# douglasbagnall/recur

Hardware: AMD Instinct MI355X
Metric: BPTT timesteps*streams/sec at 1024-hidden/256-stream (higher is better)
Workload: dtype f32; 1 GPU; text-predict multi-tap generation: hidden 1024, 256 streams/GPU, BPTT depth 20, 42 symbols, RELU, weighted momentum, lr 1e-5; streams_per_gpu=256, global_streams=256, scaling_mode=weak, parallelism=single GPU, rccl_ranks=0, exchange=none

## Files before the change

### recur_amd/csrc/k_delta_direct.h

```cpp
#pragma once
#include <hip/hip_runtime.h>
#include <stdint.h>
#include <utility>
#include "k_tiles.h"

typedef float dd_f4 __attribute__((ext_vector_type(4)));
typedef float dd_f4u __attribute__((ext_vector_type(4), aligned(4)));

struct DdArgs {
  const float *x;
  const float *e;
  const float *coef;
  const int *n_exec;
  const float *ih_scale;
  float *w, *m, *delta;
  size_t plane;
  int I, H, Scap;
  int nrows, D, uidx;
  int tm, tn;
  int rest;
  int hidden_size;
  int mode;
  int method;
  float rate, momentum, mw;
  float *ho_w, *ho_m;
  const float *ho_delta;
  float *ho_delta_out;
  unsigned ho_n4;
  float ho_rate;
  int ksplit;
  size_t kplane;
  int rgroups;
  int ho_ks;
  size_t ho_plane;
  int fast_its;
};

template <bool COLD = false> __device__ __forceinline__ dd_f4 dd_load4(const void *sbase, unsigned voff) {
  dd_f4 r;
  if constexpr (COLD) asm volatile("s_nop 4\n\tglobal_load_dwordx4 %0, %1, %2" : "=v"(r) : "v"(voff), "s"(sbase) : "memory");
  else asm volatile("global_load_dwordx4 %0, %1, %2" : "=v"(r) : "v"(voff), "s"(sbase) : "memory");
  return r;
}
template <bool COLD = false> __device__ __forceinline__ float dd_load1(const void *sbase, unsigned voff) {
  float r;
  if constexpr (COLD) asm volatile("s_nop 4\n\tglobal_load_dword %0, %1, %2" : "=v"(r) : "v"(voff), "s"(sbase) : "memory");
  else asm volatile("global_load_dword %0, %1, %2" : "=v"(r) : "v"(voff), "s"(sbase) : "memory");
  return r;
}
typedef int dd_i4 __attribute__((ext_vector_type(4)));
__device__ __forceinline__ dd_i4 dd_load4i(const void *sbase, unsigned voff) {
  dd_i4 r;
  asm volatile("s_nop 4\n\tglobal_load_dwordx4 %0, %1, %2" : "=v"(r) : "v"(voff), "s"(sbase) : "memory");
  return r;
}
template <int N> __device__ __forceinline__ void dd_flag_wait(dd_i4 (&n)[DD_FLAG_LOADS / 2], dd_f4 (&s)[DD_FLAG_LOADS / 2]) {
  static_assert(DD_FLAG_LOADS == 8, "operand list");
  asm volatile("s_waitcnt vmcnt(%8)" : "+v"(n[0]), "+v"(n[1]), "+v"(n[2]), "+v"(n[3]), "+v"(s[0]), "+v"(s[1]), "+v"(s[2]), "+v"(s[3]) : "n"(N));
}
template <int N> __device__ __forceinline__ void dd_wait3(dd_f4 &a, dd_f4 &b, float &c) {
  asm volatile("s_waitcnt vmcnt(%3)" : "+v"(a), "+v"(b), "+v"(c) : "n"(N));
}
template <int N> __device__ __forceinline__ void dd_wait4(dd_f4 &a, dd_f4 &b, float &c, float &d) {
  asm volatile("s_waitcnt vmcnt(%4)" : "+v"(a), "+v"(b), "+v"(c), "+v"(d) : "n"(N));
}
template <int N> __device__ __forceinline__ void dd_wait5(dd_f4 &a, dd_f4 &b, float &c, float &d, float &e) {
  asm volatile("s_waitcnt vmcnt(%5)" : "+v"(a), "+v"(b), "+v"(c), "+v"(d), "+v"(e) : "n"(N));
}
template <int N> __device__ __forceinline__ void dd_wait6(dd_f4 &a, dd_f4 &b, float &c, float &d, float &e, float &f) {
  asm volatile("s_waitcnt vmcnt(%6)" : "+v"(a), "+v"(b), "+v"(c), "+v"(d), "+v"(e), "+v"(f) : "n"(N));
}
template <int N> __device__ __forceinline__ void dd_wait7(dd_f4 &a, dd_f4 &b, float &c, float &d, float &e, float &f, float &g) {
  asm volatile("s_waitcnt vmcnt(%7)" : "+v"(a), "+v"(b), "+v"(c), "+v"(d), "+v"(e), "+v"(f), "+v"(g) : "n"(N));
}
template <int P> __device__ __forceinline__ void dd_drain(const dd_f4 (&a)[P], const dd_f4 (&b)[P], const float (&c)[2][P], const float (&s)[2][P], const float (&d)[P]) {
  static_assert(P == 5, "operand list");
  asm volatile("s_waitcnt vmcnt(0)"
               :
               : "v"(a[0]), "v"(a[1]), "v"(a[2]), "v"(a[3]), "v"(a[4]), "v"(b[0]), "v"(b[1]), "v"(b[2]), "v"(b[3]), "v"(b[4]),
                 "v"(c[0][0]), "v"(c[0][1]), "v"(c[0][2]), "v"(c[0][3]), "v"(c[0][4]), "v"(c[1][0]), "v"(c[1][1]), "v"(c[1][2]),
                 "v"(c[1][3]), "v"(c[1][4]), "v"(s[0][0]), "v"(s[0][1]), "v"(s[0][2]), "v"(s[0][3]), "v"(s[0][4]), "v"(s[1][0]), "v"(s[1][1]),
                 "v"(s[1][2]), "v"(s[1][3]), "v"(s[1][4]), "v"(d[0]), "v"(d[1]), "v"(d[2]), "v"(d[3]), "v"(d[4])
               : "memory");
}
template <int... Is, class F>
__device__ __forceinline__ void dd_static_for_impl(std::integer_sequence<int, Is...>, F &&f) {
  (f(std::integral_constant<int, Is>{}), ...);
}
template <int N, class F> __device__ __forceinline__ void dd_static_for(F &&f) {
  dd_static_for_impl(std::make_integer_sequence<int, N>{}, f);
}

constexpr int DD_LD = 64;
#ifndef DD_NT_STORES
#define DD_NT_STORES 1
#endif
template <int LEVEL> __device__ __forceinline__ void dd_store4(float *p, const float __attribute__((ext_vector_type(4))) & v) {
  typedef float f4u __attribute__((ext_vector_type(4), aligned(4)));
  if constexpr (DD_NT_STORES >= LEVEL) __builtin_nontemporal_store(v, reinterpret_cast<f4u *>(p));
  else *reinterpret_cast<f4u *>(p) = v;
}

#ifdef PC_STAMPS
__device__ unsigned long long g_ddir_stamps[4][8];
__device__ unsigned long long g_ddir_wave[4][8];
__device__ unsigned long long g_ddir_clk[4][4];
#define DDIR_CLOCKS(i) do { if ((blockIdx.x & 63) == 0 && threadIdx.x == 0) { g_ddir_clk[blockIdx.x >> 6][i] = __builtin_amdgcn_s_memrealtime(); g_ddir_clk[blockIdx.x >> 6][(i) + 1] = __builtin_amdgcn_s_memtime(); } } while (0)
#define DDIR_STAMP(i) do { if ((blockIdx.x & 63) == 0 && threadIdx.x == 0) g_ddir_stamps[blockIdx.x >> 6][i] = __builtin_amdgcn_s_memrealtime(); } while (0)
#else
#define DDIR_STAMP(i) do { } while (0)
#define DDIR_CLOCKS(i) do { } while (0)
#endif
struct DdNoPre {
  __device__ __forceinline__ void operator()() const {}
};
template <int NW, int P, int NPW, class PRE = DdNoPre>
__device__ __forceinline__ void dd_body(const DdArgs &a, float *lds, PRE pre = PRE{}) {
  const int wv = __builtin_amdgcn_readfirstlane((int)(threadIdx.x >> 6)), lane = threadIdx.x & 63;
  DDIR_STAMP(0);
  const int ksp = a.ksplit > 1 ? a.ksplit : 1, per_part = gridDim.x / ksp;
  const int kz = (int)blockIdx.x / per_part;
  const int L = (int)blockIdx.x - kz * per_part, xcd = L & 7, q = L >> 3;
  float *const dlt = a.delta + (size_t)kz * a.kplane;
  int mt, nt;
  if ((a.tm & 3) == 0 && (a.tn & 1) == 0) {
    const int bm = a.tm >> 2, bn = a.tn >> 1;
    mt = (xcd & 3) * bm + q % bm;
    nt = (xcd >> 2) * bn + q / bm;
  } else {
    mt = L % a.tm;
    nt = L / a.tm;
  }
  if (nt >= a.tn) return;
  const int m0 = 64 * mt, n0 = 64 * nt;
  const int I = a.I;
  const int QPS = a.nrows >> 2;
  constexpr int ST = NW / 2;
  const int n_pair = 2 * (a.D * (QPS / NW) / ksp);
  const int nf = a.fast_its > 0 ? a.fast_its : n_pair / 2;
  const bool first_of_pair = wv < ST;
  const int n_it = first_of_pair ? nf : n_pair - nf;
  const int q0 = (wv & (ST - 1)) + ST * (kz * n_pair + (first_of_pair ? 0 : nf));
  const int g_t0 = q0 / QPS, g_w0 = q0 - g_t0 * QPS;
  const unsigned voff = (unsigned)(((size_t)(lane >> 4) * I + (lane & 15) * 4) * sizeof(float));
  const int RG = a.rgroups;
  const bool has_rest = a.rest > 0 && NPW * mt < 4 * RG;
  const int rg = (a.rest + RG - 1) / RG;
  int ri[NPW], rj[NPW], rrows[NPW];
  unsigned voff_r[NPW];
  unsigned voff_s[NPW];
#pragma unroll
  for (int p = 0; p < NPW; p++) {
    const int pi = has_rest ? NPW * mt + p : 0;
    ri[p] = pi >> 2;
    rj[p] = pi & 3;
    int left = a.rest - ri[p] * rg;
    rrows[p] = has_rest ? (left < 0 ? 0 : left < rg ? left : rg) : 0;
    const int c = lane & 15;
    const int rcol = rrows[p] > 0 ? 64 * a.tm - m0 + ri[p] * rg + (c < rrows[p] ? c : rrows[p] - 1) : 0;
    voff_r[p] = (unsigned)(((size_t)(lane >> 4) * I + rcol) * sizeof(float));
    voff_s[p] = voff + (unsigned)(rj[p] * sizeof(float));
  }
  const unsigned voff_c = (unsigned)((lane >> 4) * sizeof(float));

  constexpr int CPT = 1024 / (64 * NW);
  const bool upd = a.mode == 2;

  dd_f4 fl_s[DD_FLAG_LOADS / 2];
  dd_i4 fl_n[DD_FLAG_LOADS / 2];
#pragma unroll
  for (int u = 0; u < DD_FLAG_LOADS / 2; u++) {
    int r4 = 4 * (64 * u + lane);
    r4 = r4 < a.nrows ? r4 : a.nrows - 4;
    fl_n[u] = dd_load4i(a.n_exec, (unsigned)(r4 * sizeof(int)));
    fl_s[u] = dd_load4<true>(a.ih_scale, (unsigned)(r4 * sizeof(float)));
  }

  dd_f4 ra[P], re[P];
  float rr[2][P], rs[2][P], rcf[P];
  int g_t = g_t0, g_within = g_w0;
  const float *g_xb, *g_eb, *g_cb;
  auto advance = [&]() {
    const int t = g_t < a.D ? g_t : a.D - 1;
    int slot = a.uidx - t;
    slot = slot < 0 ? slot + a.D : slot;
    const size_t ro = (size_t)(g_within << 2) * I;
    g_xb = a.x + (size_t)slot * a.plane + ro + m0;
    g_eb = a.e + (size_t)t * a.plane + ro + n0;
    g_cb = a.coef + (size_t)t * a.Scap + (g_within << 2);
    const int over = g_within + ST - QPS, neg = over >> 31;
    g_within = over + (neg & QPS);
    g_t += 1 + neg;
  };
  dd_f4 acc[4][4], racc[NPW];
#pragma unroll
  for (int p = 0; p < NPW; p++) racc[p] = dd_f4{0.f, 0.f, 0.f, 0.f};
#pragma unroll
  for (int j = 0; j < P; j++) rr[1][j] = rs[1][j] = 0.0f;
#pragma unroll
  for (int i = 0; i < 4; i++)
#pragma unroll
    for (int j = 0; j < 4; j++) acc[i][j] = dd_f4{0.f, 0.f, 0.f, 0.f};
  dd_static_for<P>([&](auto JC) {
    constexpr int j = decltype(JC)::value;
    advance();
    ra[j] = dd_load4<true>(g_xb, voff);
    re[j] = dd_load4<true>(g_eb, voff);
#pragma unroll
    for (int p = 0; p < NPW; p++) {
      rr[p][j] = dd_load1<true>(g_xb, voff_r[p]);
      rs[p][j] = dd_load1<true>(g_eb, voff_s[p]);
    }
  });
  pre();
  int ones;
  {
    DDIR_STAMP(1);
    dd_flag_wait<(2 + 2 * NPW) * P>(fl_n, fl_s);
    DDIR_STAMP(2);
    DDIR_CLOCKS(0);
    bool ok = true;
#pragma unroll
    for (int u = 0; u < DD_FLAG_LOADS / 2; u++)
#pragma unroll
      for (int k = 0; k < 4; k++) ok = ok && fl_n[u][k] == a.D && fl_s[u][k] == 1.0f;
    ones = __builtin_amdgcn_readfirstlane(__all(ok) ? 1 : 0);
  }
  auto round = [&](auto ONESC) {
    constexpr bool ONES = decltype(ONESC)::value;
    dd_static_for<P>([&](auto JC) {
      constexpr int j = decltype(JC)::value;
      constexpr int PER = 2 + 2 * NPW + (ONES ? 0 : 1);
      if constexpr (ONES && NPW == 1) dd_wait4<PER * (P - 1)>(ra[j], re[j], rr[0][j], rs[0][j]);
      else if constexpr (ONES) dd_wait6<PER * (P - 1)>(ra[j], re[j], rr[0][j], rr[1][j], rs[0][j], rs[1][j]);
      else if constexpr (NPW == 1) dd_wait5<PER * (P - 1)>(ra[j], re[j], rr[0][j], rs[0][j], rcf[j]);
      else dd_wait7<PER * (P - 1)>(ra[j], re[j], rr[0][j], rr[1][j], rs[0][j], rs[1][j], rcf[j]);
      dd_f4 fa = ra[j], fe = re[j];
      float fr[NPW], fsel[NPW];
#pragma unroll
      for (int p = 0; p < NPW; p++) {
        fr[p] = rr[p][j];
        fsel[p] = rs[p][j];
      }
      if constexpr (!ONES) {
        if constexpr (NPW == 1)
          asm volatile("v_mul_legacy_f32 %0, %5, %0\n\tv_mul_legacy_f32 %1, %5, %1\n\t"
                       "v_mul_legacy_f32 %2, %5, %2\n\tv_mul_legacy_f32 %3, %5, %3\n\tv_mul_legacy_f32 %4, %5, %4\n\ts_nop 1"
                       : "+v"(fe[0]), "+v"(fe[1]), "+v"(fe[2]), "+v"(fe[3]), "+v"(fsel[0])
                       : "v"(rcf[j]));
        else
          asm volatile("v_mul_legacy_f32 %0, %6, %0\n\tv_mul_legacy_f32 %1, %6, %1\n\t"
                       "v_mul_legacy_f32 %2, %6, %2\n\tv_mul_legacy_f32 %3, %6, %3\n\tv_mul_legacy_f32 %4, %6, %4\n\t"
                       "v_mul_legacy_f32 %5, %6, %5\n\ts_nop 1"
                       : "+v"(fe[0]), "+v"(fe[1]), "+v"(fe[2]), "+v"(fe[3]), "+v"(fsel[0]), "+v"(fsel[NPW - 1])
                       : "v"(rcf[j]));
      }
      __builtin_amdgcn_sched_barrier(0);
      advance();
#pragma unroll
      for (int i = 0; i < 4; i++)
#pragma unroll
        for (int jn = 0; jn < 4; jn++)
          acc[i][jn] = __builtin_amdgcn_mfma_f32_16x16x4f32(fa[i], fe[jn], acc[i][jn], 0, 0, 0);
#pragma unroll
      for (int p = 0; p < NPW; p++) racc[p] = __builtin_amdgcn_mfma_f32_16x16x4f32(fr[p], fsel[p], racc[p], 0, 0, 0);
#pragma unroll
      for (int g = 0; g < 16 + NPW; g++) {
        __builtin_amdgcn_sched_group_barrier(0x008, 1, 0);
        __builtin_amdgcn_sched_group_barrier(0x004, 4, 0);
      }
      __builtin_amdgcn_sched_barrier(0);
      ra[j] = dd_load4(g_xb, voff);
      re[j] = dd_load4(g_eb, voff);
#pragma unroll
      for (int p = 0; p < NPW; p++) {
        rr[p][j] = dd_load1(g_xb, voff_r[p]);
        rs[p][j] = dd_load1(g_eb, voff_s[p]);
      }
      if constexpr (!ONES) rcf[j] = dd_load1(g_cb, voff_c);
      __builtin_amdgcn_sched_barrier(0);
    });
  };
  if (ones) {
    for (int i0 = 0; i0 < n_it; i0 += P) round(std::true_type{});
    DDIR_STAMP(3);
    DDIR_CLOCKS(2);
#ifdef PC_STAMPS
    if ((blockIdx.x & 63) == 0 && lane == 0) g_ddir_wave[blockIdx.x >> 6][wv] = __builtin_amdgcn_s_memrealtime();
#endif
#pragma unroll
    for (int j = 0; j < P; j++) rcf[j] = 0.0f;
    dd_drain<P>(ra, re, rr, rs, rcf);
  } else {
#pragma unroll
    for (int j = 0; j < P; j++) rcf[j] = 0.0f;
    dd_drain<P>(ra, re, rr, rs, rcf);
    g_t = g_t0;
    g_within = g_w0;
    dd_static_for<P>([&](auto JC) {
      constexpr int j = decltype(JC)::value;
      advance();
      ra[j] = dd_load4<true>(g_xb, voff);
      re[j] = dd_load4<true>(g_eb, voff);
#pragma unroll
      for (int p = 0; p < NPW; p++) {
        rr[p][j] = dd_load1<true>(g_xb, voff_r[p]);
        rs[p][j] = dd_load1<true>(g_eb, voff_s[p]);
      }
      rcf[j] = dd_load1<true>(g_cb, voff_c);
    });
    for (int i0 = 0; i0 < n_it; i0 += P) round(std::false_type{});
    dd_drain<P>(ra, re, rr, rs, rcf);
  }

  {
    float *base = lds + (size_t)wv * 64 * DD_LD;
#pragma unroll
    for (int i = 0; i < 4; i++)
#pragma unroll
      for (int r = 0; r < 4; r++) {
        const int row = 16 * (lane >> 4) + 4 * r + i;
        *reinterpret_cast<dd_f4 *>(base + row * DD_LD + 4 * (lane & 15)) = dd_f4{acc[i][0][r], acc[i][1][r], acc[i][2][r], acc[i][3][r]};
      }
#pragma unroll
    for (int p = 0; p < NPW; p++) {
      float *rb = lds + (size_t)NW * 64 * DD_LD + (p * NW + wv) * 256;
#pragma unroll
      for (int r = 0; r < 4; r++) rb[(4 * (lane >> 4) + r) * 16 + (lane & 15)] = racc[p][r];
    }
  }
  DDIR_STAMP(4);
  __syncthreads();
  DDIR_STAMP(5);
  const bool adagrad = a.method == 4;
  auto update4 = [&](dd_f4 &W, dd_f4 &M, const dd_f4 &d, float rate) {
#pragma unroll
    for (int k = 0; k < 4; k++) {
      if (adagrad) {
        const float acc2 = M[k] + d[k] * d[k];
        W[k] += d[k] * rate / sqrtf(acc2);
        M[k] = acc2;
      } else {
        const float t = d[k] * rate, mm = M[k];
        W[k] += t + mm * a.mw;
        M[k] = (mm + t) * a.momentum;
      }
    }
  };
#pragma unroll
  for (int u = 0; u < CPT; u++) {
    const int ch = u * 64 * NW + threadIdx.x;
    const float *p = lds + (ch >> 4) * DD_LD + 4 * (ch & 15);
    dd_f4 s = *reinterpret_cast<const dd_f4 *>(p);
#pragma unroll
    for (int w2 = 1; w2 < NW; w2++) s += *reinterpret_cast<const dd_f4 *>(p + (size_t)w2 * 64 * DD_LD);
    const size_t off = (size_t)(m0 + (ch >> 4)) * a.H + n0 + 4 * (ch & 15);
    if (a.mode == 1) s += *reinterpret_cast<const dd_f4u *>(dlt + off);
    dd_store4<1>(dlt + off, s);
    if (upd) {
      dd_f4 W = *reinterpret_cast<const dd_f4u *>(a.w + off), M = *reinterpret_cast<const dd_f4u *>(a.m + off);
      update4(W, M, s, a.rate);
      dd_store4<2>(a.w + off, W);
      dd_store4<1>(a.m + off, M);
    }
  }
  auto update1 = [&](size_t off, float d, float rate, float *w, float *m) {
    if (adagrad) {
      const float acc2 = m[off] + d * d;
      w[off] += d * rate / sqrtf(acc2);
      m[off] = acc2;
      return;
    }
    const float t = d * rate, mm = m[off];
    w[off] += t + mm * a.mw;
    m[off] = (mm + t) * a.momentum;
  };
  if (has_rest && threadIdx.x < 256 * NPW) {
    const int p = threadIdx.x >> 8, t8 = threadIdx.x & 255;
    const int c = t8 >> 4, c2 = t8 & 15;
    const int pri = NPW == 1 ? ri[0] : (p ? ri[NPW - 1] : ri[0]), prj = NPW == 1 ? rj[0] : (p ? rj[NPW - 1] : rj[0]);
    const int prows = NPW == 1 ? rrows[0] : (p ? rrows[NPW - 1] : rrows[0]);
    if (c < prows) {
      const float *q = lds + (size_t)NW * 64 * DD_LD + (size_t)p * NW * 256 + t8;
      float d = q[0];
#pragma unroll
      for (int w2 = 1; w2 < NW; w2++) d += q[w2 * 256];
      const size_t off = (size_t)(64 * a.tm + pri * rg + c) * a.H + n0 + 4 * c2 + prj;
      if (a.mode == 1) d += dlt[off];
      dlt[off] = d;
      if (upd) update1(off, d, a.rate, a.w, a.m);
    }
  }
  const int hi_cols = a.H - a.hidden_size - 1;
  if (a.mode != 1 && (nt == 0 || nt == a.tn - 1)) {
    const int ncol = nt == 0 && nt == a.tn - 1 ? 1 + hi_cols : nt == 0 ? 1 : hi_cols;
    const int nrow = 64 + (mt == 0 ? a.rest : 0);
    for (int e = threadIdx.x; e < nrow * ncol; e += 64 * NW) {
      const int rr_ = e / ncol, cc = e - rr_ * ncol;
      const int row = rr_ < 64 ? m0 + rr_ : 64 * a.tm + rr_ - 64;
      const int col = (nt == 0 && cc == 0) ? -1 : a.hidden_size + (nt == 0 ? cc - 1 : cc);
      const ptrdiff_t off = (ptrdiff_t)row * a.H + col;
      dlt[off] = 0.0f;
      if (upd && adagrad) {
        a.w[off] += 0.0f * a.rate / sqrtf(a.m[off]);
      } else if (upd) {
        const float mm = a.m[off];
        a.w[off] += mm * a.mw;
        a.m[off] = mm * a.momentum;
      }
    }
  }
  if (upd && a.ho_n4) {
    const unsigned per = (a.ho_n4 + gridDim.x - 1) / gridDim.x;
    for (unsigned k = threadIdx.x; k < per; k += 64 * NW) {
      const unsigned idx = blockIdx.x * per + k;
      if (idx >= a.ho_n4) break;
      const size_t off = 4 * (size_t)idx;
      dd_f4 d = *reinterpret_cast<const dd_f4 *>(a.ho_delta + off);
      for (int z = 1; z < a.ho_ks; z++) {
        const dd_f4 t = *reinterpret_cast<const dd_f4 *>(a.ho_delta + (size_t)z * a.ho_plane + off);
        d[0] += t[0]; d[1] += t[1]; d[2] += t[2]; d[3] += t[3];
      }
      if (a.ho_delta_out) *reinterpret_cast<dd_f4 *>(a.ho_delta_out + off) = d;
      dd_f4 W = *reinterpret_cast<const dd_f4 *>(a.ho_w + off), M = *reinterpret_cast<const dd_f4 *>(a.ho_m + off);
      update4(W, M, d, a.ho_rate);
      *reinterpret_cast<dd_f4 *>(a.ho_w + off) = W;
      *reinterpret_cast<dd_f4 *>(a.ho_m + off) = M;
    }
  }
  DDIR_STAMP(6);
}

constexpr int dd_lds_bytes(int NW, int NPW = 1) { return (NW * 64 * DD_LD + NPW * NW * 256) * 4; }

#ifndef DD_BND_MARK
#define DD_BND_MARK(which) do { } while (0)
#endif
template <int NW, int P, int NPW = 1>
__global__ __launch_bounds__(64 * NW) __attribute__((amdgpu_waves_per_eu(NW / 4, NW / 4))) void k_delta_direct(DdArgs a) {
  extern __shared__ __attribute__((aligned(16))) float dd_lds[];
  __builtin_amdgcn_s_setprio(2);
  DD_BND_MARK(0);
  dd_body<NW, P, NPW>(a, dd_lds);
  DD_BND_MARK(1);
}
```

### recur_amd/csrc/kernels_bptt.hip

```cpp
#include "k_common.h"
#include "k_gemm.h"
#include "calc_plan.h"

__global__ __launch_bounds__(64) void k_bottom_error(View v, int row0, int nxp,
                                                     const unsigned char *active) {
  const RamdShape &s = v.sh;
  int j = blockIdx.x, r = row0 + j;
  int n = (active && !active[j]) ? 0 : v.b.n_exec[r];
  for (int y = threadIdx.x; y < s.bO; y += 64) {
    float sum = 0.0f;
    if (y < s.input_size)
      for (int k = 0; k < n; k++) sum += v.b.ex[((size_t)(k + 1) * s.Scap + r) * nxp + y + 1];
    v.b.berr[(size_t)r * s.bO + y] = sum;
  }
}

__global__ __launch_bounds__(256) void k_bottom_delta(View v, int row0, int nrows, int accumulate,
                                                      const unsigned char *active,
                                                      const float *carry_in, float *carry_out) {
  const RamdShape &s = v.sh;
  int e = blockIdx.x * 256 + threadIdx.x;
  if (e >= s.bI * s.bO) return;
  int yi = e / s.bO, x = e - yi * s.bO;
  float cum = carry_in[x];
  float acc = accumulate ? v.b.bdelta[e] : 0.0f;
  for (int j = 0; j < nrows; j++) {
    if (active && !active[j]) continue;
    int r = row0 + j;
    cum += v.b.berr[(size_t)r * s.bO + x];
    const float sc = v.b.ih_scale[r];
    if (sc != 1.0f && x < s.input_size) cum *= sc * sc;
    float xi = v.b.binp[(size_t)r * s.bI + yi];
    if (xi != 0.0f) acc += xi * cum;
  }
  v.b.bdelta[e] = acc;
  if (yi == 0) carry_out[x] = cum;
}

#include "k_bptt_top.h"
#include "k_bptt_extras.h"

BND_DECL(g_bnd_delta, ramd_bnd_delta_stamps)
#ifdef BND_STAMPS
#define DD_BND_MARK(which) BND_MARK(g_bnd_delta, which)
#endif
#include "k_delta_direct.h"

#ifdef PC_STAMPS
extern "C" void ramd_ddir_stamps(unsigned long long *out) {
  HIP_CHECK(hipDeviceSynchronize());
  HIP_CHECK(hipMemcpyFromSymbol(out, HIP_SYMBOL(g_ddir_stamps), sizeof(unsigned long long) * 32));
  HIP_CHECK(hipMemcpyFromSymbol(out + 32, HIP_SYMBOL(g_ddir_wave), sizeof(unsigned long long) * 32));
}
extern "C" void ramd_ddir_clocks(unsigned long long *out) {
  HIP_CHECK(hipDeviceSynchronize());
  HIP_CHECK(hipMemcpyFromSymbol(out, HIP_SYMBOL(g_ddir_clk), sizeof(unsigned long long) * 16));
}
#endif
template <int NW, int P, int NPW>
__global__ __launch_bounds__(64 * NW) __attribute__((amdgpu_waves_per_eu(NW / 4, NW / 4))) void k_delta_direct_ho(DdArgs a, View v,
                                                                                                                HoWork hw, HoApply ap) {
  extern __shared__ __attribute__((aligned(16))) float ddh_lds[];
  __builtin_amdgcn_s_setprio(2);
  BND_MARK(g_bnd_delta, 0);
#ifndef DD_HO_AT_END
#define DD_HO_AT_END 1
#endif
#if DD_HO_AT_END
  dd_body<NW, P, NPW>(a, ddh_lds);
  __syncthreads();
  chain_ho_delta<5, 8>(v, hw, ddh_lds, (int)blockIdx.x, ap);
#else
  dd_body<NW, P, NPW>(a, ddh_lds, [&]() { chain_ho_delta<5, 8>(v, hw, ddh_lds, (int)blockIdx.x, ap); });
#endif
  BND_MARK(g_bnd_delta, 1);
}

#include "k_delta_dma.h"
#include "k_bptt_small.h"


__global__ __launch_bounds__(256) void k_delta_finalize(float *delta, const float *slab,
                                                        size_t n4, size_t n, int ks,
                                                        int accumulate, int H, int hidden_size,
                                                        int rows_core, int ks_rest,
                                                        const float *rest, size_t rest_stride,
                                                        float *ho_delta, const float *ho_slab,
                                                        size_t ho_n, int ho_ks) {
  size_t q = (size_t)blockIdx.x * 256 + threadIdx.x;
  const size_t ih_threads = ((n4 + 255) / 256) * 256;
  if (q >= ih_threads) {
    size_t e = q - ih_threads;
    if (ho_slab && 4 * e < ho_n) {
      float4 a = accumulate ? ld4(ho_delta + 4 * e) : zero4();
      for (int z = 0; z < ho_ks; z++) {
        float4 t = ld4(ho_slab + (size_t)z * ho_n + 4 * e);
        a.x += t.x; a.y += t.y; a.z += t.z; a.w += t.w;
      }
      *reinterpret_cast<float4 *>(ho_delta + 4 * e) = a;
    }
    return;
  }
  if (q >= n4) return;
  const float *src = slab + 4 * q;
  size_t stride = n;
  if ((int)((4 * q) / (size_t)H) >= rows_core) {
    ks = ks_rest;
    src = rest + (4 * q - (size_t)rows_core * H);
    stride = rest_stride;
  }
  float4 a = accumulate ? ld4(delta + 4 * q) : zero4();
  float4 sum = sum_planes(src, stride, ks);
  int c = (int)((4 * q) % (size_t)H);
  a.x += (c + 0 >= 1 && c + 0 <= hidden_size) ? sum.x : 0.0f;
  a.y += (c + 1 >= 1 && c + 1 <= hidden_size) ? sum.y : 0.0f;
  a.z += (c + 2 >= 1 && c + 2 <= hidden_size) ? sum.z : 0.0f;
  a.w += (c + 3 >= 1 && c + 3 <= hidden_size) ? sum.w : 0.0f;
  *reinterpret_cast<float4 *>(delta + 4 * q) = a;
}

extern "C" void ramd_launch_pending_finalize(ramd_stream_t st_, const RamdPendingDelta *p) {
  hipStream_t st = (hipStream_t)st_;
  const size_t n4 = p->slab ? p->n / 4 : 0;
  const unsigned blocks = (unsigned)((n4 + 255) / 256) + (p->ho_slab ? (unsigned)((p->ho_n / 4 + 255) / 256) : 0u);
  if (!blocks) return;
  RAMD_LAUNCH(k_delta_finalize, dim3(blocks), dim3(256), 0, st, p->delta_out, p->slab, n4, p->n, p->ks, 0, p->H,
              p->hidden_size, p->rows_core, p->ks_rest, p->rest, p->rest_stride, p->ho_delta_out, p->ho_slab, p->ho_n,
              p->ho_ks);
}

__global__ __launch_bounds__(256) void k_err_writeback(View v, int row0, int nxp) {
  int r = row0 + blockIdx.x;
  int n = v.b.n_exec[r];
  if (n <= 0) return;
  for (int i = threadIdx.x; i < v.sh.I; i += 256) write_error_images(v, r, n, nxp, i);
}

__global__ void k_zero_f4(float *a, size_t n4) {
  size_t q = (size_t)blockIdx.x * blockDim.x + threadIdx.x;
  if (q < n4) *reinterpret_cast<float4 *>(a + 4 * q) = zero4();
}

extern "C" void ramd_launch_bottom_deltas(ramd_stream_t st_, const RamdShape *sh, RamdBuffers *b,
                                          int row0, int nrows, int accumulate,
                                          const unsigned char *active) {
  hipStream_t st = (hipStream_t)st_;
  View v = make_view(sh, b);
  RAMD_LAUNCH(k_bottom_error, dim3(nrows), dim3(64), 0, st, v, row0, ramd_nxp(sh), active);
  int n = sh->bI * sh->bO;
  const float *cin = b->bcarry + (size_t)b->bcarry_cur * sh->bO;
  float *cout = b->bcarry + (size_t)(b->bcarry_cur ^ 1) * sh->bO;
  RAMD_LAUNCH(k_bottom_delta, dim3((n + 255) / 256), dim3(256), 0, st, v, row0, nrows,
                     accumulate, active, cin, cout);
  b->bcarry_cur ^= 1;
}

extern "C" void ramd_launch_clear_deltas(ramd_stream_t st_, const RamdShape *sh,
                                         const RamdBuffers *b) {
  hipStream_t st = (hipStream_t)st_;
  size_t ih4 = (size_t)sh->I * sh->H / 4, ho4 = (size_t)sh->H * sh->O / 4;
  RAMD_LAUNCH(k_zero_f4, dim3((unsigned)((ih4 + 255) / 256)), dim3(256), 0, st, b->ih_delta, ih4);
  RAMD_LAUNCH(k_zero_f4, dim3((unsigned)((ho4 + 255) / 256)), dim3(256), 0, st, b->ho_delta, ho4);
  if (sh->bI) {
    size_t b4 = (size_t)sh->bI * sh->bO / 4, c4 = (size_t)2 * sh->bO / 4;
    RAMD_LAUNCH(k_zero_f4, dim3((unsigned)((b4 + 255) / 256)), dim3(256), 0, st, b->bdelta, b4);
    RAMD_LAUNCH(k_zero_f4, dim3((unsigned)((c4 + 255) / 256)), dim3(256), 0, st, b->bcarry, c4);
  }
}

static int g_calc_wrote_images = 0;
static void (*g_delta_half_hook)(void *ctx, int half, size_t first_float, size_t n_floats) = nullptr;
static void *g_delta_half_ctx = nullptr;
extern "C" void ramd_set_delta_half_hook(void (*hook)(void *, int, size_t, size_t), void *ctx) {
  g_delta_half_hook = hook;
  g_delta_half_ctx = ctx;
}
extern "C" int ramd_calc_wrote_images(void) {
  int w = g_calc_wrote_images;
  g_calc_wrote_images = 0;
  return w;
}

struct CalcCall {
  hipStream_t st;
  View v;
  const RamdShape *sh;
  const RamdBuffers *b;
  int row0, nrows, accumulate;
  const int *ranges;
  int range_stride;
  const unsigned char *active;
  RamdPendingDelta *defer;
  CalcPlan p;
};

static void calc_top_backprop(const CalcCall &c) {
  const RamdShape *sh = c.sh;
  const RamdBuffers *b = c.b;
  const CalcPlan &p = c.p;
  if (p.writeback_first) ramd_launch_err_writeback(c.st, sh, b, c.row0, c.nrows);
  const size_t shm = (size_t)(sh->O + sh->H) * sizeof(float);
  if (p.top == TOP_SPARSE) {
    const int alen = b->mheads_alen, ncls = sh->output_size / alen;
    const int span4 = (3 + alen + 3) / 4, ld = (4 * span4) | 1;
    raise_lds_limit<k_top_heads_partial>(96 * 1024);
    RAMD_LAUNCH(k_top_heads_partial, dim3(ncls, (sh->H + THP_ROWS - 1) / THP_ROWS), dim3(256),
                (size_t)((THP_ROWS + 32) * ld + 4) * sizeof(float), c.st, c.v, c.row0, c.nrows, c.ranges, c.range_stride, c.active,
                alen, ncls, b->mheads_part);
    RAMD_LAUNCH(k_top_heads_combine, dim3(c.nrows), dim3(THC_THREADS), 0, c.st, c.v, c.row0, c.ranges, c.range_stride, c.active,
                ncls, b->mheads_part, (p.flags & RAMD_IMAGES_PENDING) ? 1 : 0);
  } else if (p.top == TOP_HEADS) {
    const int tm = (c.nrows + 31) / 32, tn = (sh->H + 31) / 32;
    RAMD_LAUNCH(k_top_backprop_heads, dim3(tm * tn), dim3(512), (size_t)((sh->O + 15) / 16) * sizeof(unsigned), c.st, c.v,
                c.row0, c.nrows, c.ranges, c.range_stride, c.active, b->slab, p.top_nb, tm);
    RAMD_LAUNCH(k_top_backprop_scale, dim3(c.nrows), dim3(256), 0, c.st, c.v, c.row0, c.active, b->slab, p.top_nb);
  } else if (p.top == TOP_RANGED) {
    RAMD_LAUNCH(k_top_backprop_ranged, dim3(c.nrows, p.top_nb), dim3(1024), shm, c.st, c.v, c.row0, c.ranges, c.range_stride,
                c.active, b->slab);
    if (p.top_nb > 1) RAMD_LAUNCH(k_top_backprop_scale, dim3(c.nrows), dim3(256), 0, c.st, c.v, c.row0, c.active, b->slab, p.top_nb);
  } else if (p.top == TOP_PLAIN)
    RAMD_LAUNCH(k_top_backprop, dim3(c.nrows), dim3(256), shm, c.st, c.v, c.row0, c.ranges, c.range_stride, c.active);
}

struct HoOwed {
  bool gemm, sum_here;
  ProbHoDelta prob;
  int nkt, ks;
};

static HoOwed calc_top_delta(const CalcCall &c, HoWork *req, bool chain_answered) {
  const RamdShape *sh = c.sh;
  const RamdBuffers *b = c.b;
  RamdPendingDelta *defer = c.defer;
  HoOwed owed = {};
  if (c.p.ho_in_delta || (c.p.flags & RAMD_NO_HO_DELTA)) return owed;
  if (c.p.ho_asked && !chain_answered) {
    req->dst = (defer && b->ho_slab) ? b->ho_slab : b->ho_delta;
    req->active = c.active;
    req->row0 = c.row0;
    req->nrows = c.nrows;
    return owed;
  }
  if (c.p.ho_asked && req->done) {
    if (defer) {
      defer->ho_slab = req->dst == b->ho_slab ? b->ho_slab : nullptr;
      defer->ho_n = (size_t)sh->H * sh->O;
      defer->ho_ks = 1;
      defer->ho_delta_out = b->ho_delta;
    }
    return owed;
  }
  const HoGemmPlan h = ramd_plan_ho_gemm(sh, b, c.p, c.nrows, c.accumulate, c.ranges != nullptr, c.range_stride,
                                         c.active != nullptr, defer != nullptr);
  if (defer) defer->ho_slab = nullptr;
  if (h.form == HO_HEADS) {
    const int alen = b->mheads_alen, ncls = sh->output_size / alen;
    RAMD_LAUNCH(k_ho_delta_heads, dim3(ncls, (sh->H + 31) / 32), dim3(256), (size_t)(HDH_K * ((alen | 1) + 32) + 8) * sizeof(float),
                c.st, c.v, c.row0, c.nrows, c.ranges, c.range_stride, c.active, alen, ncls, c.accumulate);
    return owed;
  }
  const float *live = b->ones + c.row0;
  if (c.active) {
    RAMD_LAUNCH(k_live_mask, dim3((c.nrows + 255) / 256), dim3(256), 0, c.st, b->coef + c.row0, c.active, c.nrows);
    live = b->coef + c.row0;
  }
  const ProbHoDelta prob = {c.v, c.row0, c.nrows, live};
  if (h.form == HO_PLANES_PAIRED || h.form == HO_PAIRED_SUMMED)
    owed = {true, h.form == HO_PAIRED_SUMMED, prob, h.nkt, h.ks};
  else
    launch_gemm<true, true, ProbHoDelta>(c.st, prob, h.form == HO_PLANES ? b->ho_slab : b->slab, sh->H, sh->O, h.nkt, h.ks, T_OTHER);
  if (h.form == HO_PLANES || h.form == HO_PLANES_PAIRED) {
    defer->ho_slab = b->ho_slab;
    defer->ho_n = (size_t)sh->H * sh->O;
    defer->ho_ks = h.ks;
    defer->ho_delta_out = b->ho_delta;
  }
  if (h.form == HO_SUMMED)
    RAMD_LAUNCH(k_ho_delta_finalize, dim3((sh->H * sh->O + 255) / 256), dim3(256), 0, c.st, c.v, b->slab, h.ks, c.accumulate,
                c.range_stride ? nullptr : c.ranges);
  return owed;
}

static bool calc_settle_owed(const CalcCall &c, HoOwed &owed, bool launch_it, bool may_ride) {
  if (!owed.gemm) return false;
  if (launch_it) launch_gemm<true, true, ProbHoDelta>(c.st, owed.prob, c.b->ho_slab, c.sh->H, c.sh->O, owed.nkt, owed.ks, T_OTHER);
  owed.gemm = false;
  if (!owed.sum_here) return false;
  if (may_ride && !c.ranges) return true;
  RAMD_LAUNCH(k_ho_delta_finalize, dim3((c.sh->H * c.sh->O + 255) / 256), dim3(256), 0, c.st, c.v, c.b->ho_slab, owed.ks,
              c.accumulate, c.range_stride ? nullptr : c.ranges);
  return false;
}

static void calc_small(const CalcCall &c) {
  raise_lds_limit<k_bptt_small>(150 * 1024);
  if (c.defer) c.defer->slab = nullptr;
  int ev = timing_begin(c.st, T_CHAIN, 1);
  RAMD_LAUNCH(k_bptt_small, dim3(1), dim3(1024), c.p.small_lds, c.st, c.v, c.row0, c.accumulate, c.p.flags, c.p.nx, c.p.nxp);
  timing_end(c.st, ev);
  g_calc_wrote_images = 1;
}

static XcWork calc_xc_request(const CalcCall &c) {
  XcWork xc = {};
  if (c.p.xc_req == XC_NONE) return xc;
  xc.on = 1;
  xc.dense = c.p.xc_req == XC_DENSE;
  xc.row0 = c.row0;
  xc.nx = c.p.nx;
  xc.nxp = c.p.nxp;
  xc.active = c.active;
  xc.flags = c.p.flags;
  return xc;
}

static void calc_extras_control(const CalcCall &c, int tn_parts) {
  const RamdShape *sh = c.sh;
  const CalcPlan &p = c.p;
  const size_t shm = (size_t)(2 * sh->D + 1) * sizeof(float);
  if (p.extras == XF_CONTROL5)
    RAMD_LAUNCH((k_extras_control<5, 1024>), dim3(c.nrows), dim3(1024), shm, c.st, c.v, c.row0, c.nrows, p.nx, p.nxp, tn_parts,
                c.active, p.flags);
  else if (p.extras == XF_CONTROL8)
    RAMD_LAUNCH((k_extras_control<8, 512>), dim3(c.nrows), dim3(512), shm, c.st, c.v, c.row0, c.nrows, p.nx, p.nxp, tn_parts,
                c.active, p.flags);
  else if (p.extras == XF_CONTROL9)
    RAMD_LAUNCH((k_extras_control<9, 512>), dim3(c.nrows), dim3(512), shm, c.st, c.v, c.row0, c.nrows, p.nx, p.nxp, tn_parts,
                c.active, p.flags);
  else if (p.extras == XF_DENSE)
    ramd_launch_extras_dense(c.st, c.v, sh, c.row0, c.nrows, p.nx, p.nxp, tn_parts, 0, sh->D);
  else {
    const int M = sh->D * c.nrows;
    ProbExtras prob = {c.v, c.row0, c.nrows, p.nx};
    launch_gemm<false, false, ProbExtras>(c.st, prob, c.b->slab, M, p.nxp, (sh->H + BK - 1) / BK, p.xks, T_OTHER);
    RAMD_LAUNCH(k_extras_finalize, dim3(M), dim3(64), 0, c.st, c.v, c.row0, c.nrows, p.nx, p.nxp, p.xks, tn_parts);
  }
  if (p.extras == XF_DENSE || p.extras == XF_GEMM)
    RAMD_LAUNCH(k_bptt_control, dim3((c.nrows + 3) / 4), dim3(256), 0, c.st, c.v, c.row0, c.nrows, c.active, p.flags, p.tn);
}

struct DeltaPlanes {
  int ks, rows_core, ks_rest;
  const float *rest;
  size_t rest_stride;
  bool ho_rides;
};
static DeltaPlanes whole_planes(const CalcCall &c, int ks, int ks_rest) {
  return {ks, c.sh->I, ks_rest, c.b->slab + c.p.n, c.p.n, false};
}

static void launch_delta_finalize(const CalcCall &c, size_t first, size_t floats, int ks, int rows_core, int ks_rest, const float *rest,
                                  size_t rest_stride, const float *ho_slab, size_t ho_n, int ho_ks) {
  const size_t n4 = floats / 4;
  const unsigned blocks = (unsigned)((n4 + 255) / 256) + (ho_slab ? (unsigned)(((size_t)c.sh->H * c.sh->O / 4 + 255) / 256) : 0u);
  RAMD_LAUNCH(k_delta_finalize, dim3(blocks), dim3(256), 0, c.st, c.b->ih_delta + first, c.b->slab + first, n4, c.p.n, ks,
              c.accumulate, c.sh->H, c.sh->hidden_size, rows_core, ks_rest, rest, rest_stride, c.b->ho_delta, ho_slab, ho_n, ho_ks);
}

template <int NPW> static void launch_delta_direct(const CalcCall &c, const DdArgs &a, const HoWork *hw, const HoApply *ap) {
  const int tiles = c.p.dtm * c.p.dtn;
  if (hw) {
    raise_lds_limit<k_delta_direct_ho<DNW, DP, NPW>>(dd_lds_bytes(DNW, NPW));
    RAMD_LAUNCH((k_delta_direct_ho<DNW, DP, NPW>), dim3(tiles), dim3(64 * DNW), dd_lds_bytes(DNW, NPW), c.st, a, c.v, *hw, *ap);
  } else {
    raise_lds_limit<k_delta_direct<DNW, DP, NPW>>(dd_lds_bytes(DNW, NPW));
    RAMD_LAUNCH((k_delta_direct<DNW, DP, NPW>), dim3(c.p.dks * tiles), dim3(64 * DNW), dd_lds_bytes(DNW, NPW), c.st, a);
  }
}

static bool calc_delta_direct(const CalcCall &c, HoOwed &owed, DeltaPlanes *out) {
  const RamdShape *sh = c.sh;
  const RamdBuffers *b = c.b;
  const CalcPlan &p = c.p;
  RamdPendingDelta *defer = c.defer;
  calc_settle_owed(c, owed, true, false);
  const bool ho_planes = defer && defer->ho_slab;
  const float *ho_src = ho_planes ? defer->ho_slab : b->ho_delta;
  const bool fuse = p.direct_fuse && (ho_src || p.ho_in_delta);
  DdArgs a = {};
  a.x = b->arena + (size_t)c.row0 * sh->I;
  a.e = b->ehi + (size_t)c.row0 * sh->I + 1;
  a.coef = b->coef + c.row0;
  a.n_exec = b->n_exec + c.row0;
  a.ih_scale = b->ih_scale + c.row0;
  a.w = b->ih_w + 1;
  a.m = b->ih_m + 1;
  a.delta = b->ih_delta + 1;
  a.plane = (size_t)sh->Scap * sh->I;
  a.I = sh->I;
  a.H = sh->H;
  a.Scap = sh->Scap;
  a.nrows = c.nrows;
  a.D = sh->D;
  a.uidx = b->uniform_idx;
  a.tm = p.dtm;
  a.tn = p.dtn;
  a.rest = p.drest;
  a.rgroups = p.drg;
  a.fast_its = p.fast_its;
  a.hidden_size = sh->hidden_size;
  a.mode = fuse ? 2 : c.accumulate ? 1 : 0;
  if (p.dks > 1) {
    a.delta = b->slab + 1;
    a.ksplit = p.dks;
    a.kplane = p.n;
    a.mode = 0;
  }
  if (fuse) {
    a.rate = defer->fuse_rate;
    a.momentum = defer->fuse_momentum;
    a.mw = defer->fuse_mw;
    a.method = defer->fuse_method;
    if (!p.ho_in_delta) {
      a.ho_w = b->ho_w;
      a.ho_m = b->ho_m;
      a.ho_delta = ho_src;
      a.ho_delta_out = ho_src == b->ho_delta ? nullptr : b->ho_delta;
      a.ho_ks = ho_planes ? defer->ho_ks : 1;
      a.ho_plane = defer->ho_n;
      a.ho_n4 = (unsigned)((size_t)sh->H * sh->O / 4);
      a.ho_rate = defer->fuse_ho_rate;
    }
  }
  const bool ho_here = fuse && p.ho_in_delta;
  HoWork hw = {};
  hw.dst = b->ho_delta;
  hw.row0 = c.row0;
  hw.nrows = c.nrows;
  hw.workers = p.dtm * p.dtn;
  const HoApply ap = ho_here ? HoApply{b->ho_w, b->ho_m, defer->fuse_ho_rate, defer->fuse_momentum, defer->fuse_mw} : HoApply{};
  int ev = timing_begin(c.st, T_DELTA);
  if (p.npw == 2)
    launch_delta_direct<2>(c, a, ho_here ? &hw : nullptr, &ap);
  else
    launch_delta_direct<1>(c, a, ho_here ? &hw : nullptr, &ap);
  timing_end(c.st, ev);
  if (p.dks > 1) {
    *out = whole_planes(c, p.dks, p.ks);
    return false;
  }
  if (defer) {
    defer->slab = nullptr;
    if (fuse) {
      defer->ho_slab = nullptr;
      defer->fuse_done = 1;
    }
  }
  return true;
}

static void launch_delta_dma(const CalcCall &c, const GemmOut &o, int blocks, const DmaPlan &d, bool rest) {
  const size_t shm = (size_t)DD_STAGES * DD_STAGE_FLOATS * sizeof(float), shm_rest = shm + (size_t)DD_REST_FLOATS * sizeof(float);
  DeltaRest dr = {};
  if (rest) dr = {c.b->slab + d.rest_off, d.rest_plane, d.rest_rows, d.rows_core};
  if (!rest) {
    raise_lds_limit<k_delta_dma<0>>((int)shm);
    RAMD_LAUNCH(k_delta_dma<0>, dim3(blocks), dim3(512), shm, c.st, c.v, c.row0, c.nrows, o, dr);
  } else if (d.rest_rows <= 64) {
    raise_lds_limit<k_delta_dma<64>>((int)shm_rest);
    RAMD_LAUNCH(k_delta_dma<64>, dim3(blocks), dim3(512), shm_rest, c.st, c.v, c.row0, c.nrows, o, dr);
  } else {
    raise_lds_limit<k_delta_dma<128>>((int)shm_rest);
    RAMD_LAUNCH(k_delta_dma<128>, dim3(blocks), dim3(512), shm_rest, c.st, c.v, c.row0, c.nrows, o, dr);
  }
}

static void calc_delta_dma_halves(const CalcCall &c, const DmaPlan &d, GemmOut o, const HoOwed &owed, bool ho_direct) {
  const RamdShape *sh = c.sh;
  const size_t half_floats = (size_t)d.tmh * 128 * sh->H, up_floats = c.p.n - half_floats, ho_n = (size_t)sh->H * sh->O;
  o.tm = d.tmh;
  o.ks = d.kd2;
  int ev = timing_begin(c.st, T_DELTA, 2);
  launch_delta_dma(c, o, d.blocks2, d, false);
  launch_delta_finalize(c, 0, half_floats, d.kd2, d.tmh * 128, 0, c.b->slab, 0, nullptr, 0, 0);
  g_delta_half_hook(g_delta_half_ctx, 0, 0, half_floats);
  o.row0m = d.tmh * 128;
  launch_delta_dma(c, o, d.blocks2, d, true);
  timing_end(c.st, ev);
  if (!ho_direct) launch_gemm<true, true, ProbHoDelta>(c.st, owed.prob, c.b->ho_slab, sh->H, sh->O, owed.nkt, owed.ks, T_OTHER);
  launch_delta_finalize(c, half_floats, up_floats, d.kd2, d.rows_core - d.tmh * 128, d.kd2 * d.tmh, c.b->slab + d.rest_off,
                        d.rest_plane, ho_direct ? nullptr : c.b->ho_slab, ho_direct ? 0 : ho_n, ho_direct ? 0 : owed.ks);
  g_delta_half_hook(g_delta_half_ctx, 1, half_floats, up_floats + ho_n);
}

static bool calc_delta_dma(const CalcCall &c, HoOwed &owed, bool ho_direct, DeltaPlanes *out) {
  const RamdShape *sh = c.sh;
  const RamdBuffers *b = c.b;
  const CalcPlan &p = c.p;
  const DmaPlan d = ramd_plan_delta_dma(sh, p, c.ranges != nullptr, c.defer != nullptr, g_delta_half_hook != nullptr,
                                        (owed.gemm && owed.sum_here) || ho_direct);
  const int ncol = sh->hidden_size + 1;
  GemmOut o;
  o.slab = b->slab;
  o.M = sh->I;
  o.N = ncol;
  o.ldc = sh->H;
  o.zs = p.n;
  o.nkt = p.nkt;
  o.tm = d.tm;
  o.tn = d.tn;
  o.ks = d.kd;
  o.col0 = 1;
  o.row0m = 0;
  if (d.halves) {
    calc_delta_dma_halves(c, d, o, owed, ho_direct);
    return true;
  }
  int ev = timing_begin(c.st, T_DELTA);
  launch_delta_dma(c, o, d.blocks, d, d.rest_in);
  timing_end(c.st, ev);
  *out = {d.kd, d.rows_core, d.ks_rest, d.ks_rest ? b->slab + d.rest_off : b->slab + (size_t)d.rows_core * sh->H,
          d.ks_rest ? d.rest_plane : p.n, false};
  if (d.rest_in) {
    out->ho_rides = calc_settle_owed(c, owed, true, true);
  } else if (d.rest_rows > 0) {
    ProbDelta<true> prob = {c.v, c.row0, c.nrows, p.rtiles};
    float *rest_slab = b->slab + d.rest_off - (size_t)d.rows_core * sh->H;
    if (owed.gemm) {
      int blocks_a, blocks_b;
      GemmOut oa = make_gemm_out(b->ho_slab, sh->H, sh->O, owed.nkt, owed.ks, 0, 0, 0, &blocks_a);
      GemmOut ob = make_gemm_out(rest_slab, sh->I, ncol, p.nkt, d.ks_rest, 1, sh->H, d.rows_core, &blocks_b);
      ob.zs = d.rest_plane;
      int ev2 = timing_begin(c.st, T_DELTA);
      RAMD_LAUNCH((k_gemm_pair<ProbHoDelta, ProbDelta<true>>), dim3(blocks_a + blocks_b), dim3(256), 0, c.st, owed.prob, oa,
                  blocks_a, prob, ob);
      timing_end(c.st, ev2);
      out->ho_rides = calc_settle_owed(c, owed, false, true);
    } else {
      launch_gemm<true, true, ProbDelta<true>>(c.st, prob, rest_slab, sh->I, ncol, p.nkt, d.ks_rest, T_DELTA, 1, sh->H,
                                               d.rows_core, d.rest_plane);
    }
  }
  return false;
}

static DeltaPlanes calc_delta_generic(const CalcCall &c) {
  const RamdShape *sh = c.sh;
  const CalcPlan &p = c.p;
  const int ncol = sh->hidden_size + 1;
  if (c.b->uniform_idx >= 0) {
    ProbDelta<true> prob = {c.v, c.row0, c.nrows, p.rtiles};
    if (p.big)
      launch_gemm2<ProbDelta<true>>(c.st, prob, c.b->slab, sh->I, ncol, p.nkt, p.ks, T_DELTA, 1, sh->H);
    else
      launch_gemm<true, true, ProbDelta<true>>(c.st, prob, c.b->slab, sh->I, ncol, p.nkt, p.ks, T_DELTA, 1, sh->H);
  } else {
    ProbDelta<false> prob = {c.v, c.row0, c.nrows, p.rtiles};
    if (p.big)
      launch_gemm2<ProbDelta<false>>(c.st, prob, c.b->slab, sh->I, ncol, p.nkt, p.ks, T_DELTA, 1, sh->H);
    else
      launch_gemm<true, true, ProbDelta<false>>(c.st, prob, c.b->slab, sh->I, ncol, p.nkt, p.ks, T_DELTA, 1, sh->H);
  }
  return whole_planes(c, p.ks, p.ks);
}

static void calc_hand_over(const CalcCall &c, const DeltaPlanes &d, const HoOwed &owed) {
  RamdPendingDelta *defer = c.defer;
  if (defer && !c.accumulate) {
    defer->slab = c.b->slab;
    defer->n = c.p.n;
    defer->ks = d.ks;
    defer->H = c.sh->H;
    defer->hidden_size = c.sh->hidden_size;
    defer->rows_core = d.rows_core;
    defer->ks_rest = d.ks_rest;
    defer->rest = d.rest;
    defer->rest_stride = d.rest_stride;
    defer->delta_out = c.b->ih_delta;
    return;
  }
  if (defer) defer->slab = nullptr;
  launch_delta_finalize(c, 0, c.p.n, d.ks, d.rows_core, d.ks_rest, d.rest, d.rest_stride, d.ho_rides ? c.b->ho_slab : nullptr,
                        (size_t)c.sh->H * c.sh->O, owed.ks);
}

extern "C" void ramd_launch_calc_deltas(ramd_stream_t st_, const RamdShape *sh,
                                        const RamdBuffers *b, int row0, int nrows, int accumulate,
                                        const int *ranges, int range_stride,
                                        const unsigned char *active, unsigned flags,
                                        RamdPendingDelta *defer) {
  g_calc_wrote_images = 0;
  CalcCall c = {(hipStream_t)st_, make_view(sh, b), sh, b, row0, nrows, accumulate, ranges, range_stride, active, defer,
                ramd_plan_calc_deltas(sh, b, row0, nrows, accumulate, ranges != nullptr, range_stride, active != nullptr, flags,
                                      defer, g_delta_half_hook != nullptr)};
  calc_top_backprop(c);
  HoWork ho_req = {};
  HoOwed owed = calc_top_delta(c, &ho_req, false);
  if (c.p.small) return calc_small(c);
  XcWork xc_req = calc_xc_request(c);
  const int tn_parts = ramd_chain_steps(c.st, c.v, sh, b, row0, nrows, c.p.ho_asked ? &ho_req : nullptr, xc_req.on ? &xc_req : nullptr);
  if (c.p.ho_asked) owed = calc_top_delta(c, &ho_req, true);
  if (!xc_req.done) calc_extras_control(c, tn_parts);
  RamdBuffers own_ws;
  if (c.p.own_ws) {
    own_ws = *b;
    own_ws.slab = defer->own_slab;
    own_ws.slab_floats = defer->own_slab_floats;
    c.b = &own_ws;
  }
  const bool ho_direct = c.p.ho_asked && ho_req.done && ho_req.dst == b->ho_delta;
  DeltaPlanes planes = {};
  bool complete = false;
  if (c.p.direct_runs)
    complete = calc_delta_direct(c, owed, &planes);
  else if (c.p.dma)
    complete = calc_delta_dma(c, owed, ho_direct, &planes);
  else
    planes = calc_delta_generic(c);
  if (!complete) calc_hand_over(c, planes, owed);
}

extern "C" void ramd_launch_err_writeback(ramd_stream_t st_, const RamdShape *sh,
                                          const RamdBuffers *b, int row0, int nrows) {
  hipStream_t st = (hipStream_t)st_;
  View v = make_view(sh, b);
  RAMD_LAUNCH(k_err_writeback, dim3(nrows), dim3(256), 0, st, v, row0, ramd_nxp(sh));
}
```

Before: 1.227 million stream-timesteps/s.

## Interleave hidden-to-output delta pieces into the direct delta kernel epilogue

Replaces the separate chain_ho_delta pass, which ran after the main delta body and a block barrier, with a per-workgroup 16x16 output-layer piece. The piece's loads are issued before the LDS writeback, its MFMA is computed before the existing barrier, and its weight update is applied alongside the main update. This hides the output-layer gradient latency inside the existing epilogue instead of serialising it afterwards. It uses extra LDS and register space for the piece, and it aborts when the shapes don't fit: more pieces than tiles, or rows not divisible or above 256.

```diff
diff --git a/recur_amd/csrc/k_delta_direct.h b/recur_amd/csrc/k_delta_direct.h
--- a/recur_amd/csrc/k_delta_direct.h
+++ b/recur_amd/csrc/k_delta_direct.h
@@ -111,11 +111,15 @@
 #define DDIR_STAMP(i) do { } while (0)
 #define DDIR_CLOCKS(i) do { } while (0)
 #endif
-struct DdNoPre {
-  __device__ __forceinline__ void operator()() const {}
+struct DdNoHo {
+  static constexpr bool ON = false;
+  __device__ __forceinline__ void request(int, int) {}
+  __device__ __forceinline__ void multiply(float *, int, int) {}
+  __device__ __forceinline__ void fetch() {}
+  __device__ __forceinline__ void finish(const float *) {}
 };
-template <int NW, int P, int NPW, class PRE = DdNoPre>
-__device__ __forceinline__ void dd_body(const DdArgs &a, float *lds, PRE pre = PRE{}) {
+template <int NW, int P, int NPW, class HO = DdNoHo>
+__device__ __forceinline__ void dd_body(const DdArgs &a, float *lds, HO ho = HO{}) {
   const int wv = __builtin_amdgcn_readfirstlane((int)(threadIdx.x >> 6)), lane = threadIdx.x & 63;
   DDIR_STAMP(0);
   const int ksp = a.ksplit > 1 ? a.ksplit : 1, per_part = gridDim.x / ksp;
@@ -212,7 +216,6 @@
       rs[p][j] = dd_load1<true>(g_eb, voff_s[p]);
     }
   });
-  pre();
   int ones;
   {
     DDIR_STAMP(1);
@@ -313,6 +316,12 @@
     dd_drain<P>(ra, re, rr, rs, rcf);
   }
 
+  constexpr int HO_AREA = NW * 64 * DD_LD + NPW * NW * 256;
+  if constexpr (HO::ON) {
+    ho.request(wv, lane);
+    __builtin_amdgcn_sched_barrier(0);
+  }
+
   {
     float *base = lds + (size_t)wv * 64 * DD_LD;
 #pragma unroll
@@ -328,6 +337,11 @@
 #pragma unroll
       for (int r = 0; r < 4; r++) rb[(4 * (lane >> 4) + r) * 16 + (lane & 15)] = racc[p][r];
     }
+  }
+  if constexpr (HO::ON) {
+    __builtin_amdgcn_sched_barrier(0);
+    ho.multiply(lds + HO_AREA, wv, lane);
+    ho.fetch();
   }
   DDIR_STAMP(4);
   __syncthreads();
@@ -391,6 +405,7 @@
       if (upd) update1(off, d, a.rate, a.w, a.m);
     }
   }
+  if constexpr (HO::ON) ho.finish(lds + HO_AREA);
   const int hi_cols = a.H - a.hidden_size - 1;
   if (a.mode != 1 && (nt == 0 || nt == a.tn - 1)) {
     const int ncol = nt == 0 && nt == a.tn - 1 ? 1 + hi_cols : nt == 0 ? 1 : hi_cols;
@@ -431,7 +446,7 @@
   DDIR_STAMP(6);
 }
 
-constexpr int dd_lds_bytes(int NW, int NPW = 1) { return (NW * 64 * DD_LD + NPW * NW * 256) * 4; }
+constexpr int dd_lds_bytes(int NW, int NPW = 1, bool ho = false) { return (NW * 64 * DD_LD + NPW * NW * 256 + (ho ? NW * 256 : 0)) * 4; }
 
 #ifndef DD_BND_MARK
 #define DD_BND_MARK(which) do { } while (0)
diff --git a/recur_amd/csrc/kernels_bptt.hip b/recur_amd/csrc/kernels_bptt.hip
--- a/recur_amd/csrc/kernels_bptt.hip
+++ b/recur_amd/csrc/kernels_bptt.hip
@@ -57,22 +57,79 @@
   HIP_CHECK(hipMemcpyFromSymbol(out, HIP_SYMBOL(g_ddir_clk), sizeof(unsigned long long) * 16));
 }
 #endif
+template <int NW> struct DdHoPiece {
+  static constexpr bool ON = true;
+  static constexpr int QW = 64 / NW;
+  const float *hidden, *o_error;
+  float *dst, *w, *m;
+  int H, O, nq;
+  float rate, momentum, mw;
+  bool on, fin;
+  int h0, o0;
+  size_t off;
+  float fa[QW], fb[QW], W, M;
+  __device__ __forceinline__ DdHoPiece(const View &v, const HoWork &hw, const HoApply &ap)
+      : hidden(v.b.hidden + (size_t)hw.row0 * v.sh.H), o_error(v.b.o_error + (size_t)hw.row0 * v.sh.O), dst(hw.dst), w(ap.w),
+        m(ap.m), H(v.sh.H), O(v.sh.O), nq(hw.nrows / (4 * NW)), rate(ap.rate), momentum(ap.momentum), mw(ap.mw) {}
+  __device__ __forceinline__ void request(int wv, int lane) {
+    const int ncg = (O + 15) >> 4, p = (int)blockIdx.x;
+    on = p < ((H + 15) >> 4) * ncg;
+    h0 = on ? 16 * (p / ncg) : 0;
+    o0 = on ? 16 * (p % ncg) : 0;
+    if (!on) return;
+    const int hr = h0 + (lane & 15), oc = o0 + (lane & 15);
+    const unsigned la = (unsigned)((lane >> 4) * H + (hr < H ? hr : H - 1)), lb = (unsigned)((lane >> 4) * O + (oc < O ? oc : O - 1));
+#pragma unroll
+    for (int j = 0; j < QW; j++) {
+      const int q = j < nq ? wv + NW * j : wv;
+      fa[j] = hidden[(size_t)(4 * q) * H + la];
+      fb[j] = o_error[(size_t)(4 * q) * O + lb];
+    }
+  }
+  __device__ __forceinline__ void multiply(float *area, int wv, int lane) {
+    if (!on) return;
+    dd_f4 acc = {0.f, 0.f, 0.f, 0.f};
+#pragma unroll
+    for (int j = 0; j < QW; j++) {
+      const bool have = j < nq;
+      acc = __builtin_amdgcn_mfma_f32_16x16x4f32(have ? fa[j] : 0.0f, have ? fb[j] : 0.0f, acc, 0, 0, 0);
+    }
+    float *pb = area + wv * 256;
+#pragma unroll
+    for (int r = 0; r < 4; r++) pb[(4 * (lane >> 4) + r) * 16 + (lane & 15)] = acc[r];
+  }
+  __device__ __forceinline__ void fetch() {
+    const int t8 = (int)threadIdx.x - (64 * NW - 256), c = t8 >> 4, c2 = t8 & 15;
+    fin = on && t8 >= 0 && h0 + c < H && o0 + c2 < O;
+    off = fin ? (size_t)(h0 + c) * O + o0 + c2 : 0;
+    W = M = 0.0f;
+    if (fin && w) {
+      W = w[off];
+      M = m[off];
+    }
+  }
+  __device__ __forceinline__ void finish(const float *area) {
+    if (!fin) return;
+    const float *q = area + ((int)threadIdx.x - (64 * NW - 256));
+    float d = q[0];
+#pragma unroll
+    for (int w2 = 1; w2 < NW; w2++) d += q[w2 * 256];
+    dst[off] = d;
+    if (w) {
+      const float t = d * rate, mm = M;
+      w[off] = W + (t + mm * mw);
+      m[off] = (mm + t) * momentum;
+    }
+  }
+};
+
 template <int NW, int P, int NPW>
 __global__ __launch_bounds__(64 * NW) __attribute__((amdgpu_waves_per_eu(NW / 4, NW / 4))) void k_delta_direct_ho(DdArgs a, View v,
                                                                                                                 HoWork hw, HoApply ap) {
   extern __shared__ __attribute__((aligned(16))) float ddh_lds[];
   __builtin_amdgcn_s_setprio(2);
   BND_MARK(g_bnd_delta, 0);
-#ifndef DD_HO_AT_END
-#define DD_HO_AT_END 1
-#endif
-#if DD_HO_AT_END
-  dd_body<NW, P, NPW>(a, ddh_lds);
-  __syncthreads();
-  chain_ho_delta<5, 8>(v, hw, ddh_lds, (int)blockIdx.x, ap);
-#else
-  dd_body<NW, P, NPW>(a, ddh_lds, [&]() { chain_ho_delta<5, 8>(v, hw, ddh_lds, (int)blockIdx.x, ap); });
-#endif
+  dd_body<NW, P, NPW>(a, ddh_lds, DdHoPiece<NW>(v, hw, ap));
   BND_MARK(g_bnd_delta, 1);
 }
 
@@ -360,8 +417,15 @@
 template <int NPW> static void launch_delta_direct(const CalcCall &c, const DdArgs &a, const HoWork *hw, const HoApply *ap) {
   const int tiles = c.p.dtm * c.p.dtn;
   if (hw) {
-    raise_lds_limit<k_delta_direct_ho<DNW, DP, NPW>>(dd_lds_bytes(DNW, NPW));
-    RAMD_LAUNCH((k_delta_direct_ho<DNW, DP, NPW>), dim3(tiles), dim3(64 * DNW), dd_lds_bytes(DNW, NPW), c.st, a, c.v, *hw, *ap);
+    const int pieces = ((c.sh->H + 15) / 16) * ((c.sh->O + 15) / 16);
+    if (pieces > tiles || hw->nrows % (4 * DNW) || hw->nrows > 256) {
+      fprintf(stderr, "librecur_amd: k_delta_direct_ho: %d pieces of the top layer's delta for %d workgroups, %d streams\n", pieces,
+              tiles, hw->nrows);
+      abort();
+    }
+    constexpr int lds = dd_lds_bytes(DNW, NPW, true);
+    raise_lds_limit<k_delta_direct_ho<DNW, DP, NPW>>(lds);
+    RAMD_LAUNCH((k_delta_direct_ho<DNW, DP, NPW>), dim3(tiles), dim3(64 * DNW), lds, c.st, a, c.v, *hw, *ap);
   } else {
     raise_lds_limit<k_delta_direct<DNW, DP, NPW>>(dd_lds_bytes(DNW, NPW));
     RAMD_LAUNCH((k_delta_direct<DNW, DP, NPW>), dim3(c.p.dks * tiles), dim3(64 * DNW), dd_lds_bytes(DNW, NPW), c.st, a);
```

Measured after the change: 1.233 million stream-timesteps/s, median of 6. Within noise of the previous version (+0.5%).
